# nvlong21/Lightweight-face-detection-CenterNet

Hardware: AMD Instinct MI355X
Metric: images/sec at 640x640 batch inference (higher is better)
Workload: dtype bf16; 1 GPU; BASELINE configs[1]: batch=64 640x640 bf16 on 1 MI355X per rank, forward + top-100 peak decode; synthetic uint8 images resident in HBM, calibrated synthetic weights (seed 0); 2 context(s) per GPU, batch k on context k mod 2; batch_per_gpu=64, global_batch=64, topk=100, parallelism=dp1, contexts_per_gpu=2, input_buffers=4

## Files before the change

### lightweight-face-detection-centernet_amd/csrc/cf_stem0.hip

```cpp
#include <type_traits>
#include "cf_common.h"
#include "cf_kernels.h"
#include "cf_mx.h"
#include <vector>
#include "centerface_hip.h"

namespace cf {

typedef __attribute__((ext_vector_type(8))) __bf16 mfma_bf16x8;

static inline int slot_channel(int nb, int i) {
    int h = (i >> 2) & 1;
    int r = (i & 3) + 4 * (i >> 3);
    return nb * 32 + h * 16 + r;
}

constexpr int S0_TOH = 16, S0_TOW = 16;
constexpr int S0_NT = (S0_TOH * S0_TOW / 32) * 64;
constexpr int S0_IH = S0_TOH + 2, S0_IW = S0_TOW + 2, S0_IPX = S0_IH * S0_IW;
constexpr int S0_PH = 2 * S0_IH + 1, S0_PW = 2 * S0_IW + 1;
constexpr int S0_PROW = S0_PW * 3 + 1;

void stem0_lut(float* lut ) {
    const float mean[3] = {0.408f, 0.447f, 0.470f};
    const float stdv[3] = {0.289f, 0.274f, 0.278f};
    for (int c = 0; c < 3; ++c)
        for (int u = 0; u < 256; ++u) {
            volatile float a = (float)u / 255.0f;
            volatile float b = a - mean[c];
            lut[c * 256 + u] = b / stdv[c];
        }
}

size_t stem0_proj_bytes(int dtype) { return (size_t)(32 * elem_size(dtype) / 16 / 2) * 64 * 16; }

void stem0_pack_proj(int dtype, const float* wp, void* out_host) {
    const int P = per16(dtype), HALF = 32 * (int)elem_size(dtype) / 16 / 2;
    __builtin_memset(out_host, 0, stem0_proj_bytes(dtype));
    for (int j = 0; j < HALF; ++j)
        for (int lane = 0; lane < 64; ++lane) {
            const int i = lane & 31, h = lane >> 5, co = slot_channel(0, i);
            if (co >= 16) continue;
            char* dst = (char*)out_host + ((size_t)j * 64 + lane) * 16;
            pack_chunk(dtype, wp + co * 32 + (h * HALF + j) * P, dst);
        }
    if (dtype == 2) split_pairs_inplace(out_host, 1, HALF);
}

template <typename T> using S0Mma = CfMma<T>;

#ifdef CF_X5_TIMING
__device__ unsigned long long g_s0_stamps[8];
__device__ unsigned long long g_s0_buf[204800 * 8];
#define S0_STAMP(k) { unsigned long long t_; asm volatile("s_memtime %0\n s_waitcnt lgkmcnt(0)" : "=s"(t_) :: "memory"); s0t[k] += t_ - s0q; s0q = t_; }
#else
#define S0_STAMP(k)
#endif
template <typename T, int FMT>
__global__ __launch_bounds__(S0_NT) void stem0_kernel(Stem0Params p) {
#ifdef CF_X5_TIMING
    unsigned long long s0t[6] = {0, 0, 0, 0, 0, 0}, s0q;
    asm volatile("s_memtime %0\n s_waitcnt lgkmcnt(0)" : "=s"(s0q) :: "memory");
#endif
    constexpr int P = Elem<T>::PER16;
    constexpr bool F32 = sizeof(T) == 4;
    constexpr bool PRE = std::is_same<T, sp32_t>::value;
    constexpr int ROWB = 32 * sizeof(T) + 16;
    constexpr int HALF = 32 * sizeof(T) / 16 / 2;
    constexpr int NIB = (S0_IPX + 31) / 32;
    constexpr int NW = S0_NT / 64;
    constexpr bool DWST = PRE && FMT == CF_IN_U8_HWC_BGR;
    constexpr int PROW = DWST ? 120 : S0_PROW, XOFF = DWST ? 2 : 0;
    __shared__ __attribute__((aligned(16))) char E[S0_IPX * ROWB];
    __shared__ __attribute__((aligned(16))) T Xs[S0_PH * PROW];
    __shared__ __attribute__((aligned(16))) float Wd[9 * 32];
    __shared__ float lut[FMT == CF_IN_U8_HWC_BGR ? 768 : 1];

    const int tid = threadIdx.x, lane = tid & 63, wave = tid >> 6;
    const int pl = lane & 31, h = lane >> 5;
    const int Ho = p.H >> 1, Wo = p.W >> 1;
    const int ox0 = blockIdx.x * S0_TOW, oy0 = blockIdx.y * S0_TOH, b = blockIdx.z;


    const int iy0 = 2 * (oy0 - 1), ix0 = 2 * (ox0 - 1);
    constexpr int ECOLS = S0_PW * 3;
    constexpr int RSTEP = S0_NT / ECOLS;
    constexpr int NIT = (S0_PH + RSTEP - 1) / RSTEP;
    if constexpr (DWST) {
        constexpr int ND = (S0_PW * 3 + 2 + 3) / 4, RG = S0_NT / ND, NITD = (S0_PH + RG - 1) / RG;
        const int d = tid % ND, rg = tid / ND;
        const bool tact = rg < RG;
        const int boff = ix0 * 3 - 2 + 4 * d;
        const bool din = tact && boff >= 0 && boff + 4 <= p.W * 3;
        const int cboff = min(max(boff, 0), p.W * 3 - 4);
        float sc[4], sh[4]; bool bok[4];
#pragma unroll
        for (int i = 0; i < 4; ++i) {
            const int e = 4 * d - 2 + i;
            bok[i] = din && e >= 0 && e < S0_PW * 3;
            const int ci = (e + 3) % 3;
            sc[i] = ci == 0 ? 1.0f / (255.0f * 0.289f) : ci == 1 ? 1.0f / (255.0f * 0.274f) : 1.0f / (255.0f * 0.278f);
            sh[i] = ci == 0 ? -0.408f / 0.289f : ci == 1 ? -0.447f / 0.274f : -0.470f / 0.278f;
        }
        uint32_t v[NITD];
#pragma unroll
        for (int it = 0; it < NITD; ++it) {
            const int cy = min(max(iy0 + rg + it * RG, 0), p.H - 1);
            v[it] = *reinterpret_cast<const uint32_t*>((const uint8_t*)p.x + ((size_t)b * p.H + cy) * p.W * 3 + cboff);
        }
        for (int i = tid; i < 9 * 32; i += S0_NT) Wd[i] = p.wdw[i];
#pragma unroll
        for (int it = 0; it < NITD; ++it) {
            const int r = rg + it * RG, iy = iy0 + r;
            const bool rowok = (unsigned)iy < (unsigned)p.H;
            float f[4];
#pragma unroll
            for (int i = 0; i < 4; ++i) {
                const float u = (float)((v[it] >> (8 * i)) & 0xffu);
                f[i] = (rowok && bok[i]) ? fmaf(u, sc[i], sh[i]) : 0.0f;
            }
            if (tact && r < S0_PH) st16(reinterpret_cast<char*>(Xs) + (r * PROW + 4 * d) * 4, pack16<float>(f));
        }
    } else {
        const int e = tid % ECOLS, r0 = tid / ECOLS;
        const bool tact = r0 < RSTEP;
        const int col = e / 3, ci = e - col * 3;
        const int ix = ix0 + col;
        const bool xok = tact && (unsigned)ix < (unsigned)p.W;
        const int cx = min(max(ix, 0), p.W - 1);
        float v[NIT];
#pragma unroll
        for (int it = 0; it < NIT; ++it) {
            const int r = r0 + it * RSTEP;
            const int iy = iy0 + r;
            const bool ok = xok && r < S0_PH && (unsigned)iy < (unsigned)p.H;
            const int cy = min(max(iy, 0), p.H - 1);
            if constexpr (FMT == CF_IN_U8_HWC_BGR) {
                const uint32_t u = ((const uint8_t*)p.x)[(((size_t)b * p.H + cy) * p.W + cx) * 3 + ci];
                v[it] = __uint_as_float(ok ? (u | (uint32_t)(ci << 8)) : 0xffffffffu);
            } else {
                const float f = ((const float*)p.x)[(((size_t)b * 3 + ci) * p.H + cy) * p.W + cx];
                v[it] = ok ? f : 0.0f;
            }
        }
        if constexpr (FMT == CF_IN_U8_HWC_BGR) {
            for (int i = tid; i < 768; i += S0_NT) lut[i] = p.lut[i];
        }
        for (int i = tid; i < 9 * 32; i += S0_NT) Wd[i] = p.wdw[i];
        if constexpr (FMT == CF_IN_U8_HWC_BGR) __syncthreads();
#pragma unroll
        for (int it = 0; it < NIT; ++it) {
            const int r = r0 + it * RSTEP;
            float val = v[it];
            if constexpr (FMT == CF_IN_U8_HWC_BGR) {
                const uint32_t idx = __float_as_uint(v[it]);
                val = idx == 0xffffffffu ? 0.0f : lut[idx];
// ... 459 lines not shown
            bok[i] = din && e >= 0 && e < S0_PW * 3;
            const int ci = (e + 3) % 3;
            sc[i] = ci == 0 ? 1.0f / (255.0f * 0.289f) : ci == 1 ? 1.0f / (255.0f * 0.274f) : 1.0f / (255.0f * 0.278f);
            sh[i] = ci == 0 ? -0.408f / 0.289f : ci == 1 ? -0.447f / 0.274f : -0.470f / 0.278f;
        }
        uint32_t v[NITD];
#pragma unroll
        for (int it = 0; it < NITD; ++it) {
            const int cy = min(max(iy0 + rg + it * RG, 0), p.H - 1);
            v[it] = *reinterpret_cast<const uint32_t*>((const uint8_t*)p.x + ((size_t)b * p.H + cy) * p.W * 3 + cboff);
        }
        const bool interior = iy0 >= 0 && iy0 + S0_PH <= p.H && ix0 * 3 - 2 >= 0 && ix0 * 3 - 2 + 4 * ND <= p.W * 3;
        auto convert = [&](auto inside) {
#pragma unroll
            for (int it = 0; it < NITD; ++it) {
                const int r = rg + it * RG, iy = iy0 + r;
                const bool rowok = (unsigned)iy < (unsigned)p.H;
                float f[4];
#pragma unroll
                for (int i = 0; i < 4; ++i) {
                    const float u = (float)((v[it] >> (8 * i)) & 0xffu);
                    const float nv = fmaf(u, sc[i], sh[i]);
                    f[i] = (decltype(inside)::value || (rowok && bok[i])) ? nv : 0.0f;
                }
                if (tact && r < S0_PH) {
                    u32x2 o; o.x = pack_bf16x2(f[0], f[1]); o.y = pack_bf16x2(f[2], f[3]);
                    *reinterpret_cast<u32x2*>(reinterpret_cast<char*>(Xs) + r * (S0P_PROW * 2) + d * 8) = o;
                }
            }
        };
        if (interior) convert(std::true_type{}); else convert(std::false_type{});
    } else {
        constexpr int ECOLS = S0_PW * 3, RSTEP = S0P_NT / ECOLS, NIT = (S0_PH + RSTEP - 1) / RSTEP;
        const int e = tid % ECOLS, r0 = tid / ECOLS;
        const bool tact = r0 < RSTEP;
        const int col = e / 3, ci = e - col * 3;
        const int ix = ix0 + col;
        const bool xok = tact && (unsigned)ix < (unsigned)p.W;
        const int cx = min(max(ix, 0), p.W - 1);
        float v[NIT];
#pragma unroll
        for (int it = 0; it < NIT; ++it) {
            const int r = r0 + it * RSTEP;
            const int iy = iy0 + r;
            const bool ok = xok && r < S0_PH && (unsigned)iy < (unsigned)p.H;
            const int cy = min(max(iy, 0), p.H - 1);
            const float f = ((const float*)p.x)[(((size_t)b * 3 + ci) * p.H + cy) * p.W + cx];
            v[it] = ok ? f : 0.0f;
        }
#pragma unroll
        for (int it = 0; it < NIT; ++it) {
            const int r = r0 + it * RSTEP;
            if (tact && r < S0_PH) Xs[r * S0P_PROW + 2 + e] = (T)(pack_bf16x2(v[it], 0.0f) & 0xffffu);
        }
    }
    __syncthreads();

    u32x4 ws[2];
#pragma unroll
    for (int c = 0; c < 2; ++c) ws[c] = ld16((const char*)p.wstem + ((size_t)c * 64 + lane) * 16);
    u32x2 A[2][3][2];
    {
        const u32x2* at = reinterpret_cast<const u32x2*>(p.wdw) + lane;
#pragma unroll
        for (int q = 0; q < 2; ++q)
#pragma unroll
            for (int ky = 0; ky < 3; ++ky)
#pragma unroll
                for (int ks = 0; ks < 2; ++ks) A[q][ky][ks] = at[((q * 3 + ky) * 2 + ks) * 64];
    }
    constexpr int MAXB = (S0M_NIB + S0P_NW - 1) / S0P_NW;
    u32x4 xg[MAXB][2];
    const bool halo_inside = oy0 >= 1 && oy0 + S0_TOH + 1 <= Ho && ox0 >= 1 && ox0 + S0_TOW + 1 <= Wo;
    auto gather = [&](auto inside) {
#pragma unroll
    for (int t = 0; t < MAXB; ++t) {
        const int ib = wave + S0P_NW * t;
        const int ip = ib * 32 + pl;
        const int ipc = ip < S0M_IPX ? ip : S0M_IPX - 1;
        const int ty = ipc / S0M_IWP, txq = ipc - ty * S0M_IWP, tx = txq < S0_IW ? txq : S0_IW - 1;
        const int y = oy0 - 1 + ty, x = ox0 - 1 + tx;
        const bool inmap = decltype(inside)::value || (ip < S0M_IPX && (unsigned)y < (unsigned)Ho && (unsigned)x < (unsigned)Wo);
        const char* xp = reinterpret_cast<const char*>(Xs) + ((2 * ty) * S0P_PROW + (2 * tx) * 3 + 2) * 2;
#pragma unroll
        for (int c = 0; c < 2; ++c) {
            uint32_t w4[4];
#pragma unroll
            for (int i = 0; i < 4; ++i) {
                const int off = c == 0 ? h * (S0P_PROW * 2) + 4 * i
                                       : (h == 0 ? 2 * (S0P_PROW * 2) + 4 * i : 16 + (i < 2 ? i : 2) * (S0P_PROW * 2));
                const uint32_t v = *reinterpret_cast<const uint32_t*>(xp + off);
                w4[i] = inmap ? v : 0u;
            }
            xg[t][c].x = w4[0]; xg[t][c].y = w4[1]; xg[t][c].z = w4[2]; xg[t][c].w = w4[3];
        }
    }
    };
    if (halo_inside) gather(std::true_type{}); else gather(std::false_type{});
    __syncthreads();
#pragma unroll
    for (int t = 0; t < MAXB; ++t) {
        const int ib = wave + S0P_NW * t;
        if (ib >= S0M_NIB) break;
        f32x16 a;
#pragma unroll
        for (int r = 0; r < 16; ++r) a[r] = 0.0f;
#pragma unroll
        for (int c = 0; c < 2; ++c)
            a = __builtin_amdgcn_mfma_f32_32x32x16_bf16(__builtin_bit_cast(mfma_bf16x8, xg[t][c]),
                                                        __builtin_bit_cast(mfma_bf16x8, ws[c]), a, 0, 0, 0);
        char* ecell = E + (unsigned)(ib * 8 + h) * (unsigned)S0M_CP + pl * 8;
#pragma unroll
        for (int tq = 0; tq < 4; ++tq) {
            f32x2 u0, u1; u0.x = a[4 * tq]; u0.y = a[4 * tq + 1]; u1.x = a[4 * tq + 2]; u1.y = a[4 * tq + 3];
            const f32x2 y0 = swish2_pre(u0), y1 = swish2_pre(u1);
            u32x2 d;
            d.x = __builtin_bit_cast(uint32_t, __builtin_amdgcn_cvt_pkrtz(y0.x, y0.y));
            d.y = __builtin_bit_cast(uint32_t, __builtin_amdgcn_cvt_pkrtz(y1.x, y1.y));
            *reinterpret_cast<u32x2*>(ecell + 2 * tq * S0M_CP) = d;
        }
    }
    __syncthreads();

    static constexpr SetMap<S0_TOH, S0_TOW, S0M_IWQ> kSets{};
    const uint32_t se = kSets.v[wave * 16 + (lane & 15)];
    const int soy = (se >> 6) & 0x1ff, soxq = se & 63, kg = lane >> 4;
    f32x4 acc[8];
    mx_depthwise<3, S0M_IWQ, S0M_CP>(E + (unsigned)(soy * S0M_IWQ + soxq) * (unsigned)S0M_CP + kg * 64,
                                      reinterpret_cast<const u32x2 (*)[3][2]>(A), acc);
#pragma unroll
    for (int g = 0; g < 8; ++g)
#pragma unroll
        for (int i = 0; i < 4; i += 2) {
            f32x2 u; u.x = acc[g][i]; u.y = acc[g][i + 1];
            const f32x2 yv = swish2_pre(u);
            acc[g][i] = yv.x; acc[g][i + 1] = yv.y;
        }
    const u32x4 wpc = ld16((const char*)p.wproj + (size_t)lane * 16);
    const int gy = oy0 + soy, gx0 = ox0 + 4 * soxq;
#pragma unroll
    for (int i = 0; i < 4; ++i) {
        u32x4 d;
        d.x = packb(acc[0][i], acc[1][i]); d.y = packb(acc[2][i], acc[3][i]);
        d.z = packb(acc[4][i], acc[5][i]); d.w = packb(acc[6][i], acc[7][i]);
        f32x4 o = {0.0f, 0.0f, 0.0f, 0.0f};
        o = __builtin_amdgcn_mfma_f32_16x16x32_bf16(__builtin_bit_cast(mfma_bf16x8, wpc), __builtin_bit_cast(mfma_bf16x8, d), o, 0, 0, 0);
        if (gy < Ho && gx0 + i < Wo) {
            u32x2 ov; ov.x = packb(o[0], o[1]); ov.y = packb(o[2], o[3]);
            *reinterpret_cast<u32x2*>((T*)p.y + (((size_t)b * Ho + gy) * Wo + gx0 + i) * 16 + kg * 4) = ov;
        }
    }
}

hipError_t launch_stem0(hipStream_t s, int dtype, const Stem0Params& p) {
    if (p.B <= 0) return hipSuccess;
    const int Ho = p.H / 2, Wo = p.W / 2;
    if (p.kind & STEM0_MX) {
        if (dtype != 1) return hipErrorInvalidValue;
        dim3 grid((Wo + S0_TOW - 1) / S0_TOW, (Ho + S0_TOH - 1) / S0_TOH, p.B), blk(S0P_NT);
        set_kernel_tag("void cf::stem0_mx_kernel<%d>(cf::Stem0Params)", p.in_format);
        if (p.in_format == CF_IN_U8_HWC_BGR) hipLaunchKernelGGL((stem0_mx_kernel<CF_IN_U8_HWC_BGR>), grid, blk, 0, s, p);
        else hipLaunchKernelGGL((stem0_mx_kernel<CF_IN_F32_NCHW>), grid, blk, 0, s, p);
        return hipGetLastError();
    }
    if (p.kind & STEM0_PX) {
        if (dtype != 1) return hipErrorInvalidValue;
        dim3 grid((Wo + S0_TOW - 1) / S0_TOW, (Ho + S0_TOH - 1) / S0_TOH, p.B), blk(S0P_NT);
        set_kernel_tag("void cf::stem0_px_kernel<%d>(cf::Stem0Params)", p.in_format);
        if (p.in_format == CF_IN_U8_HWC_BGR) hipLaunchKernelGGL((stem0_px_kernel<CF_IN_U8_HWC_BGR>), grid, blk, 0, s, p);
        else hipLaunchKernelGGL((stem0_px_kernel<CF_IN_F32_NCHW>), grid, blk, 0, s, p);
        return hipGetLastError();
    }
    dim3 grid((Wo + S0_TOW - 1) / S0_TOW, (Ho + S0_TOH - 1) / S0_TOH, p.B), blk(S0_NT);
    set_kernel_tag("void cf::stem0_kernel<%s, %d>(cf::Stem0Params)", dtype == 0 ? "float" : dtype == 2 ? "sp32_t" : "unsigned short", p.in_format);
    if (dtype == 0) {
        if (p.in_format == CF_IN_U8_HWC_BGR) hipLaunchKernelGGL((stem0_kernel<float, CF_IN_U8_HWC_BGR>), grid, blk, 0, s, p);
        else hipLaunchKernelGGL((stem0_kernel<float, CF_IN_F32_NCHW>), grid, blk, 0, s, p);
    } else if (dtype == 2) {
        if (p.in_format == CF_IN_U8_HWC_BGR) hipLaunchKernelGGL((stem0_kernel<sp32_t, CF_IN_U8_HWC_BGR>), grid, blk, 0, s, p);
        else hipLaunchKernelGGL((stem0_kernel<sp32_t, CF_IN_F32_NCHW>), grid, blk, 0, s, p);
    } else {
        if (p.in_format == CF_IN_U8_HWC_BGR) hipLaunchKernelGGL((stem0_kernel<bf16_t, CF_IN_U8_HWC_BGR>), grid, blk, 0, s, p);
        else hipLaunchKernelGGL((stem0_kernel<bf16_t, CF_IN_F32_NCHW>), grid, blk, 0, s, p);
    }
    return hipGetLastError();
}

#ifdef CF_X5_TIMING
}
extern "C" int cf_debug_stem_stamps(unsigned long long* out6, int reset) {
    static unsigned long long host[204800 * 8];
    if (hipMemcpyFromSymbol(host, HIP_SYMBOL(cf::g_s0_buf), sizeof host) != hipSuccess) return -1;
    if (out6) { for (int k = 0; k < 6; ++k) out6[k] = 0; for (size_t w = 0; w < 204800; ++w) for (int k = 0; k < 6; ++k) out6[k] += host[w * 8 + k]; }
    if (reset) { static unsigned long long z[204800 * 8]; if (hipMemcpyToSymbol(HIP_SYMBOL(cf::g_s0_buf), z, sizeof z) != hipSuccess) return -1; }
    return 0;
}
namespace cf {
#endif
}
```

### lightweight-face-detection-centernet_amd/csrc/cf_uphead.hip

```cpp
#include "cf_exp.h"
#include "cf_common.h"
#include "cf_kernels.h"
#include <algorithm>
#include <atomic>
#include <cstdlib>

namespace cf {

typedef __attribute__((ext_vector_type(8))) __bf16 mfma_bf16x8;

constexpr int UH_TW = 32, UH_IW = UH_TW + 2;

template <typename T, int UH_TH, int NW>
struct Uh {
    static constexpr int P = Elem<T>::PER16;
    static constexpr int PIT = 24 * (int)sizeof(T);
    static constexpr int NC = PIT / 16, NCH = (NC + 1) / 2;
    static constexpr int CPD = 3 * NC, SPD = (CPD + 1) / 2;
    static constexpr int G = 16 / P;
    static constexpr int IH = UH_TH + 2, IPX = IH * UH_IW, NIB = (IPX + 31) / 32, MAXB = (NIB + NW - 1) / NW;
    static constexpr int T3B = NIB * 32 * PIT, WHB = 3 * SPD * 1024, RSB = NW * 2048;
    static constexpr int LDS = T3B + WHB + RSB;
};

template <typename T, bool COALESCE, int UH_TH = 8, int NW = 4, bool NT = false>
__global__ __launch_bounds__(NW * 64) void uphead_kernel(UpHeadParams p) {
    typedef Uh<T, UH_TH, NW> U;
    constexpr int P = U::P, PIT = U::PIT, NC = U::NC, NCH = U::NCH, CPD = U::CPD, SPD = U::SPD, G = U::G;
    constexpr int UH_IPX = U::IPX, UH_NIB = U::NIB, MAXB = U::MAXB;
    extern __shared__ __attribute__((aligned(16))) char smem[];
    char* T3 = smem;
    char* Wh = smem + U::T3B;
    char* Rs = Wh + U::WHB;
    const int tid = threadIdx.x, lane = tid & 63, wave = tid >> 6;
    const int pl = lane & 31, h = lane >> 5;
    unsigned tbx = blockIdx.x, tby = blockIdx.y, tbz = blockIdx.z;
    if (p.xcd) xcd_tile_order(tbx, tby, tbz);
    const int ox0 = tbx * UH_TW, oy0 = tby * UH_TH, b = tbz;

    for (int c = wave; c < U::WHB / 1024; c += NW)
        __builtin_amdgcn_global_load_lds((const __attribute__((address_space(1))) void*)((const char*)p.w0p + c * 1024 + lane * 16),
                                         (__attribute__((address_space(3))) void*)(Wh + c * 1024), 16, 0, 0);

    u32x4 wc[NCH];
#pragma unroll
    for (int j = 0; j < NCH; ++j) wc[j] = ld16((const char*)p.wcv + (size_t)(j * 64 + lane) * 16);
    u32x4 xs[MAXB][NCH], lw[MAXB][G];
    bool valid[MAXB]; int tapv[MAXB];
#pragma unroll
    for (int t = 0; t < MAXB; ++t) {
        const int ib = wave + NW * t;
        const int ip = ib * 32 + pl;
        const int ipc = ip < UH_IPX ? ip : UH_IPX - 1;
        const int ty = ipc / UH_IW, tx = ipc - ty * UH_IW;
        const int gy = oy0 - 1 + ty, gx = ox0 - 1 + tx;
        valid[t] = ib < UH_NIB && ip < UH_IPX && (unsigned)gy < (unsigned)p.h && (unsigned)gx < (unsigned)p.w;
        const int cy = min(max(gy, 0), p.h - 1), cx = min(max(gx, 0), p.w - 1);
        const char* xrow = (const char*)p.skip + (((size_t)b * p.h + cy) * p.w + cx) * PIT;
#pragma unroll
        for (int j = 0; j < NCH; ++j) xs[t][j] = ld16(xrow + min(h * NCH + j, NC - 1) * 16);
        const size_t low_row = ((size_t)b * (p.h >> 1) + (cy >> 1)) * (p.w >> 1) + (cx >> 1);
        tapv[t] = ((cy & 1) << 1) | (cx & 1);
#pragma unroll
        for (int g = 0; g < G; ++g) lw[t][g] = ld16((const char*)p.low + (low_row * 24 + min(h * 16 + g * P, 24 - P)) * sizeof(T));
    }
#pragma unroll
    for (int t = 0; t < MAXB; ++t) {
        const int ib = wave + NW * t;
        if (ib >= UH_NIB) break;
        const int ip = ib * 32 + pl;
        f32x16 acc;
#pragma unroll
        for (int r = 0; r < 16; ++r) acc[r] = 0.0f;
        mma_chain<T, NCH>(acc, [&](int j) { return wc[j]; }, [&](int j) { return (h * NCH + j) < NC ? xs[t][j] : zero16(); });
        const int tap = tapv[t];
#pragma unroll
        for (int g = 0; g < G; ++g) {
            const int ch = h * 16 + g * P;
            if (ch >= 24) break;
            float v[P], r[P];
#pragma unroll
            for (int e = 0; e < P; ++e) v[e] = relu_f(acc[g * P + e] + p.bias[ch + e]);
            unpack16<T>(lw[t][g], r);
#pragma unroll
            for (int e = 0; e < P; ++e) v[e] += relu_f(r[e] * p.upw[tap * 24 + ch + e] + p.upb[ch + e]);
            u32x4 o = pack16<T>(v);
            if (!valid[t]) o = zero16();
            st16(T3 + ip * PIT + ch * (int)sizeof(T), o);
        }
    }
    cf_sync_lds_dma();

    for (int ob = wave; ob < UH_TH * UH_TW / 32; ob += NW) {
        const int o = ob * 32 + pl;
        const int oy = o / UH_TW, ox = o - oy * UH_TW;
        f32x16 acc;
#pragma unroll
        for (int r = 0; r < 16; ++r) acc[r] = 0.0f;
#pragma unroll
        for (int dy = 0; dy < 3; ++dy) {
            const char* row = T3 + ((oy + dy) * UH_IW + ox) * PIT;
            mma_chain<T, SPD>(acc, [&](int j) { return ld16(Wh + ((dy * SPD + j) * 64 + lane) * 16); },
                              [&](int j) { const int c = h * SPD + j; u32x4 xc = ld16(row + (c < CPD ? c : CPD - 1) * 16);
                                           if (c >= CPD) xc = zero16(); return xc; });
        }
        const int gy = oy0 + oy, gx = ox0 + ox;
        if constexpr (!COALESCE) { if (gy >= p.h || gx >= p.w) continue; }
        float out[8];
#pragma unroll
        for (int r = 0; r < 4; ++r) { out[r] = acc[r] + p.b0[h * 4 + r]; out[4 + r] = acc[4 + r] + p.b0[8 + h * 4 + r]; }
        const size_t m = ((size_t)b * p.h + gy) * p.w + gx;
        const bool inmap = gy < p.h && gx < p.w;
        if (h == 0) {
            float sg = 1.0f / (1.0f + expf(-out[0]));
            sg = fminf(fmaxf(sg, 1e-4f), 1.0f - 1e-4f);
            out[0] = sg;
            if (p.hm_plane && inmap) p.hm_plane[m] = sg;
        }
        if constexpr (COALESCE) {
            char* rs = Rs + wave * 2048;
            st16(rs + pl * 64 + h * 16, pack16<float>(&out[0]));
            st16(rs + pl * 64 + 32 + h * 16, pack16<float>(&out[4]));
            __builtin_amdgcn_wave_barrier();
            if (gy < p.h) {
                char* row0 = (char*)(p.heads + (((size_t)b * p.h + gy) * p.w + ox0) * 16);
#pragma unroll
                for (int k = 0; k < 2; ++k) {
                    const int q = lane + 64 * k;
                    const u32x4 v = ld16(rs + q * 16);
                    if (ox0 + (q >> 2) < p.w) {
                        if constexpr (NT) __builtin_nontemporal_store(v, reinterpret_cast<u32x4*>(row0 + q * 16));
                        else st16(row0 + q * 16, v);
                    }
                }
            }
            __builtin_amdgcn_wave_barrier();
        }
        if constexpr (!COALESCE) {
            float* dst = p.heads + m * 16 + h * 4;
            st16(dst, pack16<float>(&out[0]));
            st16(dst + 8, pack16<float>(&out[4]));
        }
    }
}

struct UhRuns {
    typedef Uh<bf16_t, 16, 8> U;
    static constexpr int NW = 8, TH = 16, IH = TH + 2;
    static constexpr int TBF = 24 + 96 + 24 + 16;
    static constexpr int TB_OFF = U::LDS, WC_OFF = TB_OFF + TBF * 4, LDS = WC_OFF + 2048;
    static constexpr int ROW_B = UH_IW * U::PIT;
    static constexpr int SHARED_CHUNKS = 2 * ROW_B / 16;
    static_assert(U::MAXB == 3 && U::NIB == 20 && U::NCH == 2 && U::G == 2 && U::SPD == 5 && U::CPD == 9, "written out for this geometry");
    static_assert(SHARED_CHUNKS <= NW * 64 && WC_OFF % 16 == 0 && TB_OFF % 16 == 0, "one chunk per thread; 16-byte LDS reads");
};

__device__ __forceinline__ void uh_lds_barrier() { asm volatile("s_waitcnt lgkmcnt(0)\n\ts_barrier" ::: "memory"); }

typedef __amdgpu_buffer_rsrc_t uh_rsrc_t;
constexpr unsigned UH_OOB = 0x80000000u;
__device__ __forceinline__ uh_rsrc_t uh_rsrc(const void* base, int bytes) {
    return __builtin_amdgcn_make_buffer_rsrc(const_cast<void*>(base), 0, bytes, 0x00020000);
}
typedef __attribute__((ext_vector_type(4))) unsigned int uh_v4u;
__device__ __forceinline__ u32x4 uh_bload(uh_rsrc_t r, unsigned off) {
    return __builtin_bit_cast(u32x4, __builtin_amdgcn_raw_buffer_load_b128(r, (int)off, 0, 0));
}
__device__ __forceinline__ void uh_bstore_nt(const u32x4& v, uh_rsrc_t r, unsigned off) {
    __builtin_amdgcn_raw_buffer_store_b128(__builtin_bit_cast(uh_v4u, v), r, (int)off, 0, 2);
}
__device__ __forceinline__ void uh_bstore32(unsigned v, uh_rsrc_t r, unsigned off) {
    __builtin_amdgcn_raw_buffer_store_b32(v, r, (int)off, 0, 0);
}

__global__ __launch_bounds__(UhRuns::NW * 64) __attribute__((amdgpu_waves_per_eu(4)))
void uphead_runs_kernel(UpHeadParams p, int TX, int TY, unsigned tq, unsigned tr) {
    typedef UhRuns R;
    typedef R::U U;
    typedef bf16_t T;
    constexpr int PIT = U::PIT, NW = R::NW, UH_TH = R::TH;
    extern __shared__ __attribute__((aligned(16))) char smem[];
    char* T3 = smem;
    char* Wh = smem + U::T3B;
    char* Rs = Wh + U::WHB;
    float* Tb = reinterpret_cast<float*>(smem + R::TB_OFF);
    char* Wc = smem + R::WC_OFF;
    const int tid = threadIdx.x, lane = tid & 63, wave = __builtin_amdgcn_readfirstlane(tid >> 6);
    const int pl = lane & 31, h = lane >> 5;

    const unsigned G = gridDim.x, wg = blockIdx.x;
    unsigned t = wg * tq + wg * tr / G;
    const unsigned t1 = (wg + 1) * tq + (wg + 1) * tr / G;
    int b, col, row;
    { const unsigned per = (unsigned)(TX * TY), bi = t / per, rem = t - bi * per, ci = rem / (unsigned)TY;
      b = (int)bi; col = (int)ci; row = (int)(rem - ci * (unsigned)TY); }

    int tyx[3];
    const int wl = p.w >> 1;
#pragma unroll
    for (int k = 0; k < 3; ++k) {
        const int ip = (wave + NW * k) * 32 + pl;
        const int ty = ip / UH_IW, tx = ip - ty * UH_IW;
        tyx[k] = (ty << 8) | tx;
    }
    const int cell0 = (wave * 32 + pl) * PIT;
    const char* brow = T3 + (wave * UH_IW + pl) * PIT + h * (U::SPD * 16);

    u32x4 xs[3][2], lw[3][2];
    auto bounds = [&](int col_, int row_, int& ylo, int& ynum, int& xlo, int& xnum) {
        const int oy0 = row_ * UH_TH, ox0 = col_ * UH_TW;
        ylo = oy0 == 0 ? 1 : 0; ynum = min(R::IH, p.h - oy0 + 1) - ylo;
        xlo = ox0 == 0 ? 1 : 0; xnum = min(UH_IW, p.w - ox0 + 1) - xlo;
    };
    auto issue = [&](int b_, int col_, int row_, bool shared, bool any) {
        int ylo, ynum, xlo, xnum; bounds(col_, row_, ylo, ynum, xlo, xnum);
        const int oy0 = row_ * UH_TH, ox0 = col_ * UH_TW;
        const long long sb = (((long long)b_ * p.h + oy0 - 1) * p.w + ox0 - 1) * PIT;
        const long long lb = (((long long)b_ * (p.h >> 1) + (oy0 >> 1) - 1) * wl + (ox0 >> 1) - 1) * PIT;
        const uh_rsrc_t sk = uh_rsrc((const char*)p.skip + sb, any ? (R::IH * p.w + UH_IW) * PIT : 0);
        const uh_rsrc_t lo = uh_rsrc((const char*)p.low + lb, any ? ((R::IH / 2 + 1) * wl + UH_IW / 2 + 1) * PIT : 0);
#pragma unroll
        for (int k = 0; k < 3; ++k) {
            const int ty = tyx[k] >> 8, tx = tyx[k] & 255;
            const bool ok = (unsigned)(ty - ylo) < (unsigned)ynum && (unsigned)(tx - xlo) < (unsigned)xnum && !(shared && wave + NW * k < 2);
            const unsigned xo = ok ? (unsigned)((ty * p.w + tx) * PIT + h * 32) : UH_OOB;
            const unsigned lo_ = ok ? (unsigned)((((ty + 1) >> 1) * wl + ((tx + 1) >> 1)) * PIT + h * 32) : UH_OOB;
            xs[k][0] = uh_bload(sk, xo); lw[k][0] = uh_bload(lo, lo_);
            xs[k][1] = uh_bload(sk, h == 0 ? xo + 16 : UH_OOB); lw[k][1] = uh_bload(lo, h == 0 ? lo_ + 16 : UH_OOB);
        }
    };
    auto phase_a = [&](int col_, int row_, bool shared) {
        int ylo, ynum, xlo, xnum; bounds(col_, row_, ylo, ynum, xlo, xnum);
#pragma unroll
        for (int k = 0; k < 3; ++k) {
            const int ib = wave + NW * k;
            if (ib >= U::NIB) break;
            if (shared && ib < 2) continue;
            const int ty = tyx[k] >> 8, tx = tyx[k] & 255;
            const bool valid = (unsigned)(ty - ylo) < (unsigned)ynum && (unsigned)(tx - xlo) < (unsigned)xnum;
            const bool keep = !(shared && ty < 2);
            f32x16 acc;
#pragma unroll
            for (int r = 0; r < 16; ++r) acc[r] = 0.0f;
            mma_chain<T, 2>(acc, [&](int j) { return ld16(Wc + (j * 64 + lane) * 16); }, [&](int j) { return xs[k][j]; });
            const int tap = (((ty + 1) & 1) << 1) | ((tx + 1) & 1);
#pragma unroll
            for (int g = 0; g < 2; ++g) {
                const int ch = h * 16 + g * 8;
                if (ch >= 24) break;
                float v[8], r[8];
                unpack16<T>(lw[k][g], r);
#pragma unroll
                for (int q = 0; q < 8; q += 4) {
                    float bs[4], uw[4], ub[4];
                    unpack16<float>(ld16(Tb + ch + q), bs);
                    unpack16<float>(ld16(Tb + 24 + tap * 24 + ch + q), uw);
                    unpack16<float>(ld16(Tb + 120 + ch + q), ub);
#pragma unroll
                    for (int e = 0; e < 4; ++e) v[q + e] = relu_f(acc[g * 8 + q + e] + bs[e]);
#pragma unroll
                    for (int e = 0; e < 4; ++e) v[q + e] += relu_f(r[q + e] * uw[e] + ub[e]);
                    __builtin_amdgcn_sched_barrier(0);
                }
                u32x4 o = pack16<T>(v);
                if (!valid) o = zero16();
                if (keep) st16(T3 + cell0 + k * (NW * 32 * PIT) + ch * (int)sizeof(T), o);
            }
        }
    };

    issue(b, col, row, false, true);
    for (int c = wave; c < U::WHB / 1024; c += NW)
        __builtin_amdgcn_global_load_lds((const __attribute__((address_space(1))) void*)((const char*)p.w0p + c * 1024 + lane * 16),
                                         (__attribute__((address_space(3))) void*)(Wh + c * 1024), 16, 0, 0);
    if (wave < 2)
        __builtin_amdgcn_global_load_lds((const __attribute__((address_space(1))) void*)((const char*)p.wcv + wave * 1024 + lane * 16),
                                         (__attribute__((address_space(3))) void*)(Wc + wave * 1024), 16, 0, 0);
    if (tid < R::TBF) Tb[tid] = tid < 24 ? p.bias[tid] : tid < 120 ? p.upw[tid - 24] : tid < 144 ? p.upb[tid - 120] : p.b0[tid - 144];

    asm volatile("s_waitcnt vmcnt(0)" ::: "memory");
    uh_lds_barrier();
    phase_a(col, row, false);
    for (;;) {
        uh_lds_barrier();

        const bool more = t + 1 < t1;
        int nb = b, ncol = col, nrow = row + 1;
        bool nshared = more;
        if (nrow == TY) { nrow = 0; nshared = false; if (++ncol == TX) { ncol = 0; ++nb; } }
        issue(nb, ncol, nrow, nshared, more);

        const int ox0 = col * UH_TW, oy0 = row * UH_TH;
        const int wcells = min(UH_TW, p.w - ox0);
#pragma unroll
        for (int i = 0; i < 2; ++i) {
            const int oy = wave + NW * i;
            f32x16 acc;
#pragma unroll
            for (int r = 0; r < 16; ++r) acc[r] = 0.0f;
#pragma unroll
            for (int dy = 0; dy < 3; ++dy) {
                const char* rp = brow + (NW * i + dy) * R::ROW_B;
                mma_chain<T, 5>(acc, [&](int j) { return ld16(Wh + ((dy * 5 + j) * 64 + lane) * 16); },
                                [&](int j) { u32x4 xc = ld16(rp + j * 16); if (j == 4 && h) xc = zero16(); return xc; });
            }
            const int gy = oy0 + oy;
            float b0a[4], b0b[4], out[8];
            unpack16<float>(ld16(Tb + 144 + h * 4), b0a); unpack16<float>(ld16(Tb + 152 + h * 4), b0b);
#pragma unroll
            for (int r = 0; r < 4; ++r) { out[r] = acc[r] + b0a[r]; out[4 + r] = acc[4 + r] + b0b[r]; }
            if (h == 0) {
                float sg = 1.0f / (1.0f + expf(-out[0]));
                sg = fminf(fmaxf(sg, 1e-4f), 1.0f - 1e-4f);
                out[0] = sg;
            }
            const size_t mrow = ((size_t)b * p.h + gy) * p.w + ox0;
            const int ncell = gy < p.h ? wcells : 0;
            uh_bstore32(__float_as_uint(out[0]), uh_rsrc(p.hm_plane + mrow, p.hm_plane ? ncell * 4 : 0), h == 0 ? (unsigned)(pl * 4) : UH_OOB);
            char* rs = Rs + wave * 2048;
            st16(rs + pl * 64 + h * 16, pack16<float>(&out[0]));
            st16(rs + pl * 64 + 32 + h * 16, pack16<float>(&out[4]));
            __builtin_amdgcn_wave_barrier();
            const uh_rsrc_t hr = uh_rsrc(p.heads + mrow * 16, ncell * 64);
#pragma unroll
            for (int k = 0; k < 2; ++k) {
                const int q = lane + 64 * k;
                uh_bstore_nt(ld16(rs + q * 16), hr, (unsigned)(q * 16));
            }
            __builtin_amdgcn_wave_barrier();
        }
        if (!more) break;
        u32x4 keep2 = zero16();
        const bool copies = nshared && tid < R::SHARED_CHUNKS;
        if (copies) keep2 = ld16(T3 + (R::IH - 2) * R::ROW_B + tid * 16);
        uh_lds_barrier();
        if (copies) st16(T3 + tid * 16, keep2);
        b = nb; col = ncol; row = nrow; ++t;
        phase_a(col, row, nshared);
    }
}

template <typename T, bool CO, int TH, int NW, bool NT>
static hipError_t uphead_launch_t(hipStream_t s, const UpHeadParams& q) {
    typedef Uh<T, TH, NW> U;
    dim3 grid((q.w + UH_TW - 1) / UH_TW, (q.h + TH - 1) / TH, q.B), blk(NW * 64);
    set_kernel_tag("void cf::uphead_kernel<%s, %s, %d, %d, %s>(cf::UpHeadParams)", type_tag<T>(), CO ? "true" : "false", TH, NW, NT ? "true" : "false");
    return launch_lds<uphead_kernel<T, CO, TH, NW, NT>>(grid, blk, U::LDS, s, q);
}

static int uphead_slots() {
    static std::atomic<int> cus[32];
    int dev = 0; (void)hipGetDevice(&dev);
    std::atomic<int>& slot = cus[dev & 31];
    int n = slot.load(std::memory_order_relaxed);
    if (n <= 0) {
        if (hipDeviceGetAttribute(&n, hipDeviceAttributeMultiprocessorCount, dev) != hipSuccess || n <= 0) n = 1;
        slot.store(n, std::memory_order_relaxed);
    }
    return 2 * std::min(n, 16384);
}

static hipError_t uphead_runs_launch(hipStream_t s, const UpHeadParams& q) {
    const int TX = (q.w + UH_TW - 1) / UH_TW, TY = (q.h + UhRuns::TH - 1) / UhRuns::TH;
    const long long T = (long long)TX * TY * q.B;
    if (T > 0x7fffffffLL) return hipErrorInvalidValue;
    const unsigned G = (unsigned)std::min<long long>(T, uphead_slots());
    set_kernel_tag("cf::uphead_runs_kernel(cf::UpHeadParams, int, int, unsigned int, unsigned int)");
    return launch_lds<uphead_runs_kernel>(dim3(G), dim3(UhRuns::NW * 64), UhRuns::LDS, s, q, TX, TY, (unsigned)(T / G), (unsigned)(T % G));
}

hipError_t launch_uphead(hipStream_t s, int dtype, const UpHeadParams& p) {
    if (p.B <= 0) return hipSuccess;
    static const bool xcd_on = cf_ab_int("CF_UH_XCD", 0) >= 1;
    UpHeadParams q = p; q.xcd = xcd_on ? 1 : 0;
#include CF_EXP_INC(cf_uphead_0)
    if (dtype == 1) return uphead_runs_launch(s, q);
    if (dtype == 2) return uphead_launch_t<sp32_t, true, 8, 8, true>(s, q);
    return uphead_launch_t<float, true, 8, 4, true>(s, q);
}

}
```

Before: 53880 images/s.

## Add persistent run-based stem0 kernel reusing halo rows between vertical tiles

Adds a persistent stem0 kernel in which each workgroup walks a contiguous run of tiles down a column. It keeps the expanded halo rows in LDS so the next tile skips recomputing them, and it prefetches the next tile's input pixels while the depthwise stage runs. The goal is to cut launch and tail overhead and remove redundant halo work in the first layer. The uphead run helpers move into a shared header. The cost is more complex synchronisation and a fixed grid sized at five workgroups per CU.

```diff
diff --git a/lightweight-face-detection-centernet_amd/csrc/cf_runs.h b/lightweight-face-detection-centernet_amd/csrc/cf_runs.h
--- /dev/null
+++ b/lightweight-face-detection-centernet_amd/csrc/cf_runs.h
@@ -0,0 +1,44 @@
+#pragma once
+#include <algorithm>
+#include <atomic>
+#include "cf_common.h"
+
+namespace cf {
+
+static inline int runs_cu_count() {
+    static std::atomic<int> cus[32];
+    int dev = 0; (void)hipGetDevice(&dev);
+    std::atomic<int>& slot = cus[dev & 31];
+    int n = slot.load(std::memory_order_relaxed);
+    if (n <= 0) {
+        if (hipDeviceGetAttribute(&n, hipDeviceAttributeMultiprocessorCount, dev) != hipSuccess || n <= 0) n = 1;
+        slot.store(n, std::memory_order_relaxed);
+    }
+    return std::min(n, 16384);
+}
+
+struct RunSplit { unsigned G, tq, tr; };
+static inline bool run_split(long long T, int slots, RunSplit& r) {
+    if (T <= 0 || T > 0x7fffffffLL || slots <= 0) return false;
+    r.G = (unsigned)std::min<long long>(T, slots);
+    r.tq = (unsigned)(T / r.G); r.tr = (unsigned)(T % r.G);
+    return true;
+}
+
+__device__ __forceinline__ void run_range(unsigned wg, unsigned G, unsigned tq, unsigned tr, unsigned& t0, unsigned& t1) {
+    t0 = wg * tq + wg * tr / G;
+    t1 = (wg + 1) * tq + (wg + 1) * tr / G;
+}
+
+__device__ __forceinline__ void run_tile(unsigned t, int TX, int TY, int& b, int& col, int& row) {
+    const unsigned per = (unsigned)(TX * TY), bi = t / per, rem = t - bi * per, ci = rem / (unsigned)TY;
+    b = (int)bi; col = (int)ci; row = (int)(rem - ci * (unsigned)TY);
+}
+
+__device__ __forceinline__ unsigned run_xcd_order(unsigned wg, unsigned G) {
+    return (G & 7u) == 0u ? (wg & 7u) * (G >> 3) + (wg >> 3) : wg;
+}
+
+__device__ __forceinline__ void runs_lds_barrier() { asm volatile("s_waitcnt lgkmcnt(0)\n\ts_barrier" ::: "memory"); }
+
+}
diff --git a/lightweight-face-detection-centernet_amd/csrc/cf_stem0.hip b/lightweight-face-detection-centernet_amd/csrc/cf_stem0.hip
--- a/lightweight-face-detection-centernet_amd/csrc/cf_stem0.hip
+++ b/lightweight-face-detection-centernet_amd/csrc/cf_stem0.hip
@@ -2,6 +2,7 @@
 #include "cf_common.h"
 #include "cf_kernels.h"
 #include "cf_mx.h"
+#include "cf_runs.h"
 #include <vector>
 #include "centerface_hip.h"
 
@@ -767,11 +768,220 @@
     }
 }
 
+constexpr int S0R_KEEP_CELL = 16 * S0M_IWQ;
+constexpr int S0R_KEEP_CHUNKS = 2 * S0M_IWQ * S0M_CP / 16;
+constexpr int S0R_NIB_SHARED = (S0_TOH * S0M_IWQ) / 8;
+static_assert((S0_TOH * S0M_IWQ) % 8 == 0 && S0R_KEEP_CHUNKS <= S0P_NT && S0_PH * S0P_PROW * 2 <= S0R_KEEP_CELL * S0M_CP,
+              "rows 2-17 are whole blocks; one piece per thread; the patch ends below the kept rows");
+constexpr int S0R_AT_BYTES = 2 * 3 * 2 * 64 * 8;
+constexpr int S0R_CELLS = S0_IH * S0M_IWQ;
+static_assert(S0R_AT_BYTES % (8 * S0P_NT) == 0, "whole passes of the workgroup");
+static_assert((S0R_CELLS * S0M_CP + S0R_AT_BYTES + 1279) / 1280 * 5 <= 128, "five workgroups per CU by LDS (1280-byte pieces of 160 KB)");
+constexpr int S0R_WGS_PER_CU = 5;
+
+__global__ __launch_bounds__(S0P_NT) __attribute__((amdgpu_waves_per_eu(S0R_WGS_PER_CU)))
+void stem0_mx_kernel_runs(Stem0Params p, int TX, int TY, unsigned tq, unsigned tr) {
+    typedef bf16_t T;
+    __shared__ __attribute__((aligned(16))) char E[S0R_CELLS * S0M_CP];
+    __shared__ __attribute__((aligned(16))) char At[S0R_AT_BYTES];
+    T* Xs = reinterpret_cast<T*>(E);
+
+    const int tid0 = threadIdx.x;
+    const int wave = __builtin_amdgcn_readfirstlane(tid0 >> 6);
+    const int Ho = p.H >> 1, Wo = p.W >> 1;
+
+    unsigned wg = blockIdx.x;
+    if (p.kind & STEM0_XCD) wg = run_xcd_order(wg, gridDim.x);
+    unsigned t, t1;
+    run_range(wg, gridDim.x, tq, tr, t, t1);
+    int b, col, row;
+    run_tile(t, TX, TY, b, col, row);
+
+    constexpr int ND = S0P_ND, RG = S0P_NT / ND, NITD = (S0_PH + RG - 1) / RG;
+    uint32_t v[NITD];
+    auto issue = [&](int tid, int b_, int col_, int row_, bool shared_) {
+        const int d = tid % ND, rg = tid / ND;
+        const int iy0 = 2 * (row_ * S0_TOH - 1) + (shared_ ? 4 : 0), ix0 = 2 * (col_ * S0_TOW - 1);
+        const int cboff = min(max(ix0 * 3 - 2 + 4 * d, 0), p.W * 3 - 4);
+        const uint8_t* img = (const uint8_t*)p.x + (size_t)b_ * p.H * p.W * 3 + cboff;
+#pragma unroll
+        for (int it = 0; it < NITD; ++it) {
+            const int cy = min(max(iy0 + rg + it * RG, 0), p.H - 1);
+            v[it] = *reinterpret_cast<const uint32_t*>(img + (size_t)cy * p.W * 3);
+        }
+    };
+    issue(tid0, b, col, row, false);
+#pragma unroll
+    for (int i = 0; i < S0R_AT_BYTES / 8 / S0P_NT; ++i)
+        reinterpret_cast<u32x2*>(At)[tid0 + i * S0P_NT] = reinterpret_cast<const u32x2*>(p.wdw)[tid0 + i * S0P_NT];
+    static constexpr SetMap<S0_TOH, S0_TOW, S0M_IWQ> kSets{};
+
+    constexpr int MAXB = (S0M_NIB + S0P_NW - 1) / S0P_NW;
+    bool shared = false;
+    u32x4 keep;
+    keep = __builtin_nondeterministic_value(keep);
+    static_assert((S0R_KEEP_CELL * S0M_CP + S0R_KEEP_CHUNKS * 16) == S0R_CELLS * S0M_CP, "the kept rows are the end of E");
+    for (unsigned k = 0;; ++k) {
+        int lane;
+        asm volatile("v_mbcnt_lo_u32_b32 %0, -1, 0\n\tv_mbcnt_hi_u32_b32 %0, -1, %0" : "=v"(lane));
+        const int tid = wave * 64 + lane, pl = lane & 31, h = lane >> 5;
+        const uint32_t se = kSets.v[wave * 16 + (lane & 15)];
+        const int d = tid % ND, rg = tid / ND;
+        const bool tact = rg < RG;
+        float sc[4], sh[4];
+        const int ci0 = d + 1 - 3 * (((d + 1) * 43) >> 7);
+#pragma unroll
+        for (int i = 0; i < 4; ++i) {
+            const int ci = ci0 + i >= 3 ? ci0 + i - 3 : ci0 + i;
+            sc[i] = ci == 0 ? 1.0f / (255.0f * 0.289f) : ci == 1 ? 1.0f / (255.0f * 0.274f) : 1.0f / (255.0f * 0.278f);
+            sh[i] = ci == 0 ? -0.408f / 0.289f : ci == 1 ? -0.447f / 0.274f : -0.470f / 0.278f;
+        }
+        const int soy = (se >> 6) & 0x1ff, soxq = se & 63, kg = lane >> 4;
+        const char* dwb = E + (unsigned)(soy * S0M_IWQ + soxq) * (unsigned)S0M_CP + kg * 64;
+        const int ox0 = col * S0_TOW, oy0 = row * S0_TOH;
+        const int rofs = shared ? 4 : 0;
+        {
+            const int iy0 = 2 * (oy0 - 1), ix0 = 2 * (ox0 - 1);
+            const int boff = ix0 * 3 - 2 + 4 * d;
+            const bool din = tact && boff >= 0 && boff + 4 <= p.W * 3;
+            const bool interior = iy0 >= 0 && iy0 + S0_PH <= p.H && ix0 * 3 - 2 >= 0 && ix0 * 3 - 2 + 4 * ND <= p.W * 3;
+            auto convert = [&](auto inside) {
+#pragma unroll
+                for (int it = 0; it < NITD; ++it) {
+                    const int r = rofs + rg + it * RG, iy = iy0 + r;
+                    const bool rowok = (unsigned)iy < (unsigned)p.H;
+                    float f[4];
+#pragma unroll
+                    for (int i = 0; i < 4; ++i) {
+                        const int e = 4 * d - 2 + i;
+                        const float u = (float)((v[it] >> (8 * i)) & 0xffu);
+                        const float nv = fmaf(u, sc[i], sh[i]);
+                        f[i] = (decltype(inside)::value || (rowok && din && e >= 0 && e < S0_PW * 3)) ? nv : 0.0f;
+                    }
+                    if (tact && r < S0_PH) {
+                        u32x2 o; o.x = pack_bf16x2(f[0], f[1]); o.y = pack_bf16x2(f[2], f[3]);
+                        *reinterpret_cast<u32x2*>(reinterpret_cast<char*>(Xs) + r * (S0P_PROW * 2) + d * 8) = o;
+                    }
+                }
+            };
+            if (interior) convert(std::true_type{}); else convert(std::false_type{});
+        }
+        runs_lds_barrier();
+
+        u32x4 ws[2];
+#pragma unroll
+        for (int c = 0; c < 2; ++c) ws[c] = ld16((const char*)p.wstem + ((size_t)c * 64 + lane) * 16);
+        const int wv = (wave + (int)k) & (S0P_NW - 1);
+        const int nblk = shared ? S0R_NIB_SHARED : S0M_NIB, cell0 = shared ? 2 * S0M_IWQ : 0;
+        u32x4 xg[MAXB][2];
+        const bool halo_inside = oy0 >= 1 && oy0 + S0_TOH + 1 <= Ho && ox0 >= 1 && ox0 + S0_TOW + 1 <= Wo;
+        auto gather = [&](auto inside) {
+#pragma unroll
+            for (int tb = 0; tb < MAXB; ++tb) {
+                const int ib = wv + S0P_NW * tb;
+                if (ib >= nblk) break;
+                const int ip = cell0 * 4 + ib * 32 + pl;
+                const int ipc = ip < S0M_IPX ? ip : S0M_IPX - 1;
+                const int ty = ipc / S0M_IWP, txq = ipc - ty * S0M_IWP, tx = txq < S0_IW ? txq : S0_IW - 1;
+                const int y = oy0 - 1 + ty, x = ox0 - 1 + tx;
+                const bool inmap = decltype(inside)::value || (ip < S0M_IPX && (unsigned)y < (unsigned)Ho && (unsigned)x < (unsigned)Wo);
+                const char* xp = reinterpret_cast<const char*>(Xs) + ((2 * ty) * S0P_PROW + (2 * tx) * 3 + 2) * 2;
+#pragma unroll
+                for (int c = 0; c < 2; ++c) {
+                    uint32_t w4[4];
+#pragma unroll
+                    for (int i = 0; i < 4; ++i) {
+                        const int off = c == 0 ? h * (S0P_PROW * 2) + 4 * i
+                                               : (h == 0 ? 2 * (S0P_PROW * 2) + 4 * i : 16 + (i < 2 ? i : 2) * (S0P_PROW * 2));
+                        const uint32_t xv = *reinterpret_cast<const uint32_t*>(xp + off);
+                        w4[i] = inmap ? xv : 0u;
+                    }
+                    xg[tb][c].x = w4[0]; xg[tb][c].y = w4[1]; xg[tb][c].z = w4[2]; xg[tb][c].w = w4[3];
+                }
+            }
+        };
+        if (halo_inside) gather(std::true_type{}); else gather(std::false_type{});
+        runs_lds_barrier();
+        if (shared && tid < S0R_KEEP_CHUNKS) st16(E + tid * 16, keep);
+#pragma unroll
+        for (int tb = 0; tb < MAXB; ++tb) {
+            const int ib = wv + S0P_NW * tb;
+            if (ib >= nblk) break;
+            f32x16 a;
+#pragma unroll
+            for (int r = 0; r < 16; ++r) a[r] = 0.0f;
+#pragma unroll
+            for (int c = 0; c < 2; ++c)
+                a = __builtin_amdgcn_mfma_f32_32x32x16_bf16(__builtin_bit_cast(mfma_bf16x8, xg[tb][c]),
+                                                            __builtin_bit_cast(mfma_bf16x8, ws[c]), a, 0, 0, 0);
+            char* ecell = E + (unsigned)(cell0 + ib * 8 + h) * (unsigned)S0M_CP + pl * 8;
+            const int nq = min(4, (S0R_CELLS - cell0 - ib * 8) / 2);
+#pragma unroll
+            for (int tq4 = 0; tq4 < 4; ++tq4) {
+                if (tq4 >= nq) break;
+                f32x2 u0, u1; u0.x = a[4 * tq4]; u0.y = a[4 * tq4 + 1]; u1.x = a[4 * tq4 + 2]; u1.y = a[4 * tq4 + 3];
+                const f32x2 y0 = swish2_pre(u0), y1 = swish2_pre(u1);
+                u32x2 dd;
+                dd.x = __builtin_bit_cast(uint32_t, __builtin_amdgcn_cvt_pkrtz(y0.x, y0.y));
+                dd.y = __builtin_bit_cast(uint32_t, __builtin_amdgcn_cvt_pkrtz(y1.x, y1.y));
+                *reinterpret_cast<u32x2*>(ecell + 2 * tq4 * S0M_CP) = dd;
+            }
+        }
+        runs_lds_barrier();
+
+        const bool more = t + 1 < t1;
+        int nb = b, ncol = col, nrow = row + 1;
+        bool nshared = more;
+        if (nrow == TY) { nrow = 0; nshared = false; if (++ncol == TX) { ncol = 0; ++nb; } }
+
+        f32x4 acc[8];
+        mx_depthwise_lds<3, S0M_IWQ, S0M_CP>(dwb, At + lane * 8, acc);
+        if (more) issue(tid, nb, ncol, nrow, nshared); else issue(tid, b, col, row, false);
+        const u32x4 wpc = ld16((const char*)p.wproj + (size_t)lane * 16);
+#pragma unroll
+        for (int g = 0; g < 8; ++g)
+#pragma unroll
+            for (int i = 0; i < 4; i += 2) {
+                f32x2 u; u.x = acc[g][i]; u.y = acc[g][i + 1];
+                const f32x2 yv = swish2_pre(u);
+                acc[g][i] = yv.x; acc[g][i + 1] = yv.y;
+            }
+        const int gy = oy0 + soy, gx0 = ox0 + 4 * soxq;
+#pragma unroll
+        for (int i = 0; i < 4; ++i) {
+            u32x4 dd;
+            dd.x = packb(acc[0][i], acc[1][i]); dd.y = packb(acc[2][i], acc[3][i]);
+            dd.z = packb(acc[4][i], acc[5][i]); dd.w = packb(acc[6][i], acc[7][i]);
+            f32x4 o = {0.0f, 0.0f, 0.0f, 0.0f};
+            o = __builtin_amdgcn_mfma_f32_16x16x32_bf16(__builtin_bit_cast(mfma_bf16x8, wpc), __builtin_bit_cast(mfma_bf16x8, dd), o, 0, 0, 0);
+            if (gy < Ho && gx0 + i < Wo) {
+                u32x2 ov; ov.x = packb(o[0], o[1]); ov.y = packb(o[2], o[3]);
+                *reinterpret_cast<u32x2*>((T*)p.y + (((size_t)b * Ho + gy) * Wo + gx0 + i) * 16 + kg * 4) = ov;
+            }
+        }
+        if (!more) break;
+        keep = ld16(E + S0R_KEEP_CELL * S0M_CP + min(tid, S0R_KEEP_CHUNKS - 1) * 16);
+        runs_lds_barrier();
+        b = nb; col = ncol; row = nrow; shared = nshared; ++t;
+    }
+}
+
+static hipError_t stem0_runs_launch(hipStream_t s, const Stem0Params& p) {
+    const int TX = (p.W / 2 + S0_TOW - 1) / S0_TOW, TY = (p.H / 2 + S0_TOH - 1) / S0_TOH;
+    RunSplit r;
+    if (!run_split((long long)TX * TY * p.B, S0R_WGS_PER_CU * runs_cu_count(), r)) return hipErrorInvalidValue;
+    set_kernel_tag("cf::stem0_mx_kernel_runs(cf::Stem0Params, int, int, unsigned int, unsigned int)");
+    hipLaunchKernelGGL(stem0_mx_kernel_runs, dim3(r.G), dim3(S0P_NT), 0, s, p, TX, TY, r.tq, r.tr);
+    return hipGetLastError();
+}
+
 hipError_t launch_stem0(hipStream_t s, int dtype, const Stem0Params& p) {
     if (p.B <= 0) return hipSuccess;
     const int Ho = p.H / 2, Wo = p.W / 2;
     if (p.kind & STEM0_MX) {
         if (dtype != 1) return hipErrorInvalidValue;
+        static const int runs = cf_ab_int("CF_STEM_RUNS", 1);
+        if (p.in_format == CF_IN_U8_HWC_BGR && runs >= 1) return stem0_runs_launch(s, p);
         dim3 grid((Wo + S0_TOW - 1) / S0_TOW, (Ho + S0_TOH - 1) / S0_TOH, p.B), blk(S0P_NT);
         set_kernel_tag("void cf::stem0_mx_kernel<%d>(cf::Stem0Params)", p.in_format);
         if (p.in_format == CF_IN_U8_HWC_BGR) hipLaunchKernelGGL((stem0_mx_kernel<CF_IN_U8_HWC_BGR>), grid, blk, 0, s, p);
diff --git a/lightweight-face-detection-centernet_amd/csrc/cf_uphead.hip b/lightweight-face-detection-centernet_amd/csrc/cf_uphead.hip
--- a/lightweight-face-detection-centernet_amd/csrc/cf_uphead.hip
+++ b/lightweight-face-detection-centernet_amd/csrc/cf_uphead.hip
@@ -1,8 +1,8 @@
 #include "cf_exp.h"
 #include "cf_common.h"
 #include "cf_kernels.h"
+#include "cf_runs.h"
 #include <algorithm>
-#include <atomic>
 #include <cstdlib>
 
 namespace cf {
@@ -155,7 +155,7 @@
     static_assert(SHARED_CHUNKS <= NW * 64 && WC_OFF % 16 == 0 && TB_OFF % 16 == 0, "one chunk per thread; 16-byte LDS reads");
 };
 
-__device__ __forceinline__ void uh_lds_barrier() { asm volatile("s_waitcnt lgkmcnt(0)\n\ts_barrier" ::: "memory"); }
+__device__ __forceinline__ void uh_lds_barrier() { runs_lds_barrier(); }
 
 typedef __amdgpu_buffer_rsrc_t uh_rsrc_t;
 constexpr unsigned UH_OOB = 0x80000000u;
@@ -188,12 +188,10 @@
     const int tid = threadIdx.x, lane = tid & 63, wave = __builtin_amdgcn_readfirstlane(tid >> 6);
     const int pl = lane & 31, h = lane >> 5;
 
-    const unsigned G = gridDim.x, wg = blockIdx.x;
-    unsigned t = wg * tq + wg * tr / G;
-    const unsigned t1 = (wg + 1) * tq + (wg + 1) * tr / G;
+    unsigned t, t1;
+    run_range(blockIdx.x, gridDim.x, tq, tr, t, t1);
     int b, col, row;
-    { const unsigned per = (unsigned)(TX * TY), bi = t / per, rem = t - bi * per, ci = rem / (unsigned)TY;
-      b = (int)bi; col = (int)ci; row = (int)(rem - ci * (unsigned)TY); }
+    run_tile(t, TX, TY, b, col, row);
 
     int tyx[3];
     const int wl = p.w >> 1;
@@ -348,25 +346,14 @@
     return launch_lds<uphead_kernel<T, CO, TH, NW, NT>>(grid, blk, U::LDS, s, q);
 }
 
-static int uphead_slots() {
-    static std::atomic<int> cus[32];
-    int dev = 0; (void)hipGetDevice(&dev);
-    std::atomic<int>& slot = cus[dev & 31];
-    int n = slot.load(std::memory_order_relaxed);
-    if (n <= 0) {
-        if (hipDeviceGetAttribute(&n, hipDeviceAttributeMultiprocessorCount, dev) != hipSuccess || n <= 0) n = 1;
-        slot.store(n, std::memory_order_relaxed);
-    }
-    return 2 * std::min(n, 16384);
-}
+static int uphead_slots() { return 2 * runs_cu_count(); }
 
 static hipError_t uphead_runs_launch(hipStream_t s, const UpHeadParams& q) {
     const int TX = (q.w + UH_TW - 1) / UH_TW, TY = (q.h + UhRuns::TH - 1) / UhRuns::TH;
-    const long long T = (long long)TX * TY * q.B;
-    if (T > 0x7fffffffLL) return hipErrorInvalidValue;
-    const unsigned G = (unsigned)std::min<long long>(T, uphead_slots());
+    RunSplit r;
+    if (!run_split((long long)TX * TY * q.B, uphead_slots(), r)) return hipErrorInvalidValue;
     set_kernel_tag("cf::uphead_runs_kernel(cf::UpHeadParams, int, int, unsigned int, unsigned int)");
-    return launch_lds<uphead_runs_kernel>(dim3(G), dim3(UhRuns::NW * 64), UhRuns::LDS, s, q, TX, TY, (unsigned)(T / G), (unsigned)(T % G));
+    return launch_lds<uphead_runs_kernel>(dim3(r.G), dim3(UhRuns::NW * 64), UhRuns::LDS, s, q, TX, TY, r.tq, r.tr);
 }
 
 hipError_t launch_uphead(hipStream_t s, int dtype, const UpHeadParams& p) {
```

New measurement: 54030 images/s (median of 5 runs). About the same (+0.3%).
